# Consensys/gnark

Measured on AMD Instinct MI355X. Metric: G1 MSM throughput, BN254, 2^24 scalar-muls on one GPU (Groth16 proofs/s at 2^24 constraints in 'groth16'), higher is better.
Workload: dtype u64 Montgomery limbs in memory; 29/28-bit limbs, v_mad_u64_u32 (32x32+64) in registers

## Files before the change

gnark_amd/_lib.py:

```python
from __future__ import annotations

import ctypes as C
import os

_HERE = os.path.dirname(os.path.abspath(__file__))
DEFAULT_PATH = os.path.join(_HERE, "libgnark_amd.so")

GA_OK = 0
BN254, BLS12_381 = 0, 1
G1, G2 = 0, 1
BASES_ON_DEVICE, SCALARS_ON_DEVICE, SCALARS_MONTGOMERY, TABLE_BATCHED = 0x1, 0x2, 0x4, 0x10
RESULT_ON_DEVICE, RESULT_BITREVERSED, CHECK_CURVE_ONLY = 0x20, 0x40, 0x80
POINT_OK, POINT_OFF_CURVE, POINT_NOT_IN_SUBGROUP = 0, 1, 2
VECTOR_ON_DEVICE = BASES_ON_DEVICE
SCALE_EACH, SCALE_ONE, SCALE_POWERS = 0, 1, 2
FFT_FORWARD, FFT_INVERSE = 0, 1
DIF, DIT = 0, 1


class GnarkAmdError(RuntimeError):
    pass


class G16Key(C.Structure):
# ... 104 lines not shown
    "ga_g16_h_chain": (C.c_int, [_P, _P, C.c_uint64, _P]),
    "ga_g16_h_chain_dev": (C.c_int, [_P, _P, C.c_uint64]),
    "ga_g16_h_combine": (C.c_int, [_P, _P, _P, _P]),
    "ga_g16_z_partial": (C.c_int, [_P, _P, _P]),
    "ga_g16_prove_multi": (C.c_int, [C.POINTER(_P), C.c_uint32, _P, _P, _P, _P, C.c_uint64, C.c_uint64, _P, _P, _P]),
    "ga_g16_pk_read_mem": (C.c_int, [_P, C.c_int, _P, C.c_size_t, C.c_int32, C.c_uint32, C.c_uint32, _P, C.c_uint64, C.POINTER(_P), C.POINTER(C.c_uint64)]),
    "ga_g16_pk_read_fd": (C.c_int, [_P, C.c_int, C.c_int, C.c_int32, C.c_uint32, C.c_uint32, _P, C.c_uint64, C.POINTER(_P), C.POINTER(C.c_uint64)]),
    "ga_g16_pk_read_mem_checked": (C.c_int, [_P, C.c_int, _P, C.c_size_t, C.c_int32, C.c_uint32, C.c_uint32, _P, C.c_uint64, C.POINTER(_P), C.POINTER(C.c_uint64)]),
    "ga_g16_pk_read_fd_checked": (C.c_int, [_P, C.c_int, C.c_int, C.c_int32, C.c_uint32, C.c_uint32, _P, C.c_uint64, C.POINTER(_P), C.POINTER(C.c_uint64)]),
    "ga_g16_key_write_fd": (C.c_int, [_P, C.POINTER(G16Key), C.c_int, C.c_int, C.POINTER(C.c_uint64)]),
    "ga_g16_proof_unmarshal": (C.c_int, [C.c_int, _P, C.c_size_t, _P, _P, C.c_uint32, C.POINTER(C.c_uint32), _P, C.POINTER(C.c_size_t)]),
    "ga_point_unmarshal": (C.c_int, [C.c_int, C.c_int, _P, C.c_size_t, _P, C.POINTER(C.c_size_t)]),
    "ga_g16_proof_marshal": (C.c_int, [C.c_int, _P, _P, C.c_size_t, C.POINTER(C.c_size_t)]),
    "ga_g16_commit": (C.c_int, [_P, C.c_uint32, _P, C.c_uint64, _P, _P]),
    "ga_g16_fold_pok": (C.c_int, [C.c_int, _P, C.c_uint64, _P, _P]),
    "ga_hash_to_field": (C.c_int, [C.c_int, _P, C.c_size_t, _P, C.c_size_t, C.c_uint32, _P]),
    "ga_expand_message_xmd": (C.c_int, [_P, C.c_size_t, _P, C.c_size_t, C.c_size_t, _P]),
    "ga_g16_proof_marshal_bsb22": (C.c_int, [C.c_int, _P, _P, C.c_uint32, _P, _P, C.c_size_t, C.POINTER(C.c_size_t)]),
    "ga_g16_proof_marshal_raw": (C.c_int, [C.c_int, _P, _P, C.c_uint32, _P, _P, C.c_size_t, C.POINTER(C.c_size_t)]),
    "ga_g1_marshal_uncompressed": (C.c_int, [C.c_int, _P, _P, C.c_size_t, C.POINTER(C.c_size_t)]),
    "ga_profile_enable": (C.c_int, [_P, C.c_int]),
    "ga_profile_reset": (C.c_int, [_P]),
    "ga_profile_read": (C.c_int, [_P, C.c_char_p, C.c_size_t]),
    "ga_gen_bases": (C.c_int, [_P, C.c_int, C.c_int, C.c_uint64, C.c_size_t, _P, _P]),
    "ga_gen_bases_at": (C.c_int, [_P, C.c_int, C.c_int, C.c_uint64, C.c_uint64, C.c_size_t, _P, _P]),
    "ga_gen_scalars": (C.c_int, [_P, C.c_int, C.c_uint64, C.c_size_t, _P]),
    "ga_fr_dot": (C.c_int, [_P, C.c_int, _P, _P, C.c_size_t, _P]),
    "ga_generator_mul": (C.c_int, [C.c_int, C.c_int, _P, _P]),
    "ga_microbench": (C.c_int, [_P, C.c_char_p, C.c_size_t]),
    "ga_clock_probe": (C.c_int, [_P, C.c_uint32, C.POINTER(C.c_double)]),
}

EXPORTED_SYMBOLS = tuple(_PROTOS)


class Library:

    def __init__(self, path: str = DEFAULT_PATH):
        if not os.path.exists(path):
            raise GnarkAmdError(
                f"{path} not found: build the HIP library first "
                "(`python -c 'import __graft_entry__ as g; g.build()'` or `make -C gnark_amd/csrc -j8`). "
                "gnark_amd has no CPU fallback.")
        self.path = path
        self.dll = C.CDLL(path)
        for name, (res, args) in _PROTOS.items():
# ... 19 lines not shown
```

gnark_amd/csrc/abi.hip:

```cpp
#include <stdarg.h>
#include <stdlib.h>

#include <memory>
#include <new>
#include <vector>

#include "hostops.hip.h"

namespace ga {

static thread_local char g_err[1024] = "";

void set_error(const char* fmt, ...) {
    va_list ap;
    va_start(ap, fmt);
    vsnprintf(g_err, sizeof(g_err), fmt, ap);
    va_end(ap);
}
const char* get_error() { return g_err; }

int abi_exception_code(const char* entry) noexcept {
    try {
        throw;
    } catch (const std::bad_alloc&) {
// ... 77 lines not shown
    std::lock_guard<std::mutex> g(scratch_mu);
    auto it = scratch.find(key);
    if (it != scratch.end() && it->second.bytes >= bytes) {
        *out = it->second.p;
        return GA_OK;
    }
    if (it != scratch.end()) {
        hipFree(it->second.p);
        scratch.erase(it);
    }
    void* p = nullptr;
    const size_t slack = bytes / 8 < (64u << 20) ? bytes / 8 : (size_t)(64u << 20);
    size_t want = bytes + slack + 256;
    hipError_t e = device_malloc(&p, want);
    if (e != hipSuccess) {
        set_error("device scratch '%s': device_malloc(%zu) failed: %s", key, want, device_malloc_error(e));
        return GA_ERR_NOMEM;
    }
    scratch[key] = ScratchBuf{p, want, lane};
    *out = p;
    return GA_OK;
}

void Ctx::scratch_free_all() {
    std::lock_guard<std::mutex> g(scratch_mu);
    for (auto& kv : scratch) hipFree(kv.second.p);
    scratch.clear();
}

void Ctx::scratch_free_lanes(int first_lane) {
    std::lock_guard<std::mutex> g(scratch_mu);
    for (auto it = scratch.begin(); it != scratch.end();) {
        if (it->second.lane >= first_lane) {
            hipFree(it->second.p);
            it = scratch.erase(it);
        } else
            ++it;
    }
}

static uint64_t env_u64(const char* name, uint64_t dflt) {
    const char* e = getenv(name);
    return e ? strtoull(e, nullptr, 10) : dflt;
}
static int env_int(const char* name, int dflt) {
    const char* e = getenv(name);
// ... 16 lines not shown
    put64(g16_table_budget_pct, env_u64("GA_G16_TABLE_BUDGET_PCT", 0));
    put(g16_split, (int)env_u64("GA_G16_SPLIT", 1));
    put(g16_batch_tables, (int)env_u64("GA_G16_BATCH_TABLES", 1));
    put(ntt_wave_local, (int)env_u64("GA_NTT_WAVE_LOCAL", 1));
    put(ntt_direct, (int)env_u64("GA_NTT_DIRECT", 1));
    put(table_c, (int)env_u64("GA_TABLE_C", 0));
    put(msm_exact_redo, (int)env_u64("GA_MSM_EXACT_REDO", 0));
    put64(msm_fuse_min, env_u64("GA_MSM_FUSE_MIN", 1ull << 21));
    put64(msm_task_exact_min, env_u64("GA_MSM_TASK_EXACT_MIN", 1ull << 25));
    put(msm_xcd, (int)env_u64("GA_MSM_XCD", 3));
    {
        const uint64_t g = env_u64("GA_MSM_P1_GRID", 512);
        put64(msm_p1_grid, g ? g : 1);
    }
    {
        const char* e = getenv("GA_FAULT_THROW");
        put64(fault_throw, (e && *e) ? fnv1a(e) : 0);
    }
    put(fault_lane2_nomem, (int)env_u64("GA_FAULT_LANE2_NOMEM", 0));
    const int grp = (int)env_u64("GA_MSM_GROUP", 0);
    put(msm_group, (grp >= 2 && grp <= 256 && (grp & (grp - 1)) == 0) ? grp : 0);
    const uint64_t seg = env_u64("GA_MSM_MIN_SEG", 256);
    if (seg >= 32) put64(msm_min_seg, seg);
    g_table_c = table_c.load();
}

typedef CtxLock Lock;

static uint32_t env_segment(const char* name) {
    const uint64_t v = env_u64(name, 0);
    return (uint32_t)(v < (1u << 20) ? v : (1u << 20));
}

static bool abi_curve_ok(int curve) {
    if (curve == GA_BN254 || curve == GA_BLS12_381) return true;
    set_error("%s: unknown curve id %d", current_entry(), curve);
    return false;
}
static bool abi_curve_group_ok(int curve, int group) {
    if ((curve == GA_BN254 || curve == GA_BLS12_381) && (group == GA_G1 || group == GA_G2)) return true;
    set_error("%s: unknown curve id %d or group id %d", current_entry(), curve, group);
    return false;
}
static bool abi_range_ok(size_t n, uint64_t first) {
    if ((uint64_t)n <= (1ull << 32) && (n == 0 || first <= UINT64_MAX - (uint64_t)n + 1)) return true;
    set_error("%s: n = %zu above 2^32, or first + n above 2^64", current_entry(), n);
// ... 96 lines not shown

const char* ga_last_error(void) { return get_error(); }
const char* ga_version(void) { return "gnark_amd 0.1 (gfx950; Groth16/PLONK prover kernels: MSM G1/G2, NTT; BN254, BLS12-381)"; }

int ga_device_count(int* count) try {
    GA_ABI_ENTRY();
    GA_HIP_CHECK(hipGetDeviceCount(count));
    return GA_OK;
} GA_ABI_CATCH

int ga_ctx_create(int device, ga_ctx** out) try {
    GA_ABI_ENTRY();
    int count = 0;
    hipError_t e = hipGetDeviceCount(&count);
    if (e != hipSuccess || count <= 0) {
        set_error("no HIP device available (%s); libgnark_amd has no CPU fallback", e == hipSuccess ? "count=0" : hipGetErrorString(e));
        return GA_ERR_HIP;
    }
    if (device < 0 || device >= count) {
        set_error("device %d out of range (have %d)", device, count);
        return GA_ERR_INVALID;
    }
    GA_HIP_CHECK(hipSetDevice(device));
    {
        hipDeviceProp_t prop;
        GA_HIP_CHECK(hipGetDeviceProperties(&prop, device));
        if (prop.warpSize != 64) {
            set_error("device %d runs %d-lane wavefronts; libgnark_amd's kernels need 64 (gfx950)", device, prop.warpSize);
            return GA_ERR_INVALID;
        }
    }
    Ctx* c = new Ctx();
    c->device = device;
    hipStream_t* slots[3 + GA_NUM_LANES] = {&c->lane_stream[0], &c->lane_stream[1], &c->lane_stream[2], &c->lane_stream[3],
                                            &c->copy_stream, &c->slot_stream[0], &c->slot_stream[1]};
    for (int k = 0; k < 3 + GA_NUM_LANES; k++) {
        hipError_t se = hipStreamCreateWithFlags(slots[k], hipStreamNonBlocking);
        if (se != hipSuccess) {
            set_error("hipStreamCreate failed: %s", hipGetErrorString(se));
            for (int q = 0; q < k; q++) hipStreamDestroy(*slots[q]);
            delete c;
            return GA_ERR_HIP;
        }
    }
    c->stream = c->lane_stream[0];
    c->tun.read_env();
    *out = reinterpret_cast<ga_ctx*>(c);
    return GA_OK;
} GA_ABI_CATCH

void ga_ctx_destroy(ga_ctx* h) try {
    GA_ABI_ENTRY();
    if (!h) return;
    Ctx* c = reinterpret_cast<Ctx*>(h);
    hipSetDevice(c->device);
    for (int l = 0; l < GA_NUM_LANES; l++) hipStreamSynchronize(c->lane_stream[l]);
// ... 868 lines not shown
    }
    c->stages.clear();
    return GA_OK;
} GA_ABI_CATCH

int ga_profile_read(ga_ctx* h, char* buf, size_t cap) try {
    GA_ABI_ENTRY();
    Ctx* c = reinterpret_cast<Ctx*>(h);
    Lock l(c);
    GA_HIP_CHECK(hipStreamSynchronize(c->stream));
    std::string out;
    for (auto& s : c->stages) {
        float ms = 0;
        if (hipEventElapsedTime(&ms, s.a, s.b) != hipSuccess) ms = -1;
        char tmp[160];
        snprintf(tmp, sizeof(tmp), "%s=%.6f;", s.name.c_str(), ms);
        out += tmp;
    }
    if (!buf || cap == 0) return GA_ERR_INVALID;
    snprintf(buf, cap, "%s", out.c_str());
    return GA_OK;
} GA_ABI_CATCH

int ga_gen_bases(ga_ctx* h, int curve, int group, uint64_t seed, size_t n, void* bases_dev, void* dlogs_dev) try {
    GA_ABI_ENTRY();
    Ctx* c = reinterpret_cast<Ctx*>(h);
    Lock l(c);
    GA_DISPATCH_CURVE(curve, GA_DISPATCH_GROUP(group, GA_CHECK((util_gen_bases<C, G>(c, seed, n, bases_dev, dlogs_dev)))));
    GA_HIP_CHECK(hipStreamSynchronize(c->stream));
    return GA_OK;
} GA_ABI_CATCH

int ga_gen_bases_at(ga_ctx* h, int curve, int group, uint64_t seed, uint64_t first, size_t n, void* bases_dev, void* dlogs_dev) try {
    GA_ABI_ENTRY();
    Ctx* c = reinterpret_cast<Ctx*>(h);
    Lock l(c);
    GA_DISPATCH_CURVE(curve, GA_DISPATCH_GROUP(group, GA_CHECK((util_gen_bases<C, G>(c, seed, n, bases_dev, dlogs_dev, first)))));
    GA_HIP_CHECK(hipStreamSynchronize(c->stream));
    return GA_OK;
} GA_ABI_CATCH

int ga_gen_scalars(ga_ctx* h, int curve, uint64_t seed, size_t n, void* scalars_dev) try {
    GA_ABI_ENTRY();
    Ctx* c = reinterpret_cast<Ctx*>(h);
    Lock l(c);
    GA_DISPATCH_CURVE(curve, GA_CHECK(util_gen_scalars<C>(c, seed, n, scalars_dev)));
// ... 62 lines not shown
```

gnark_amd/csrc/common.hip.h:

```cpp
#pragma once
#include <hip/hip_runtime.h>
#include <stdint.h>
#include <stdio.h>
#include <string.h>

#include <chrono>
#include <condition_variable>
#include <atomic>
#include <map>
#include <mutex>
#include <set>
#include <string>
#include <vector>

#include "../../include/gnark_amd.h"
#include "ec.hip.h"

namespace ga {

#if defined(__HIP_DEVICE_COMPILE__) && !defined(__GFX9__)
#error "libgnark_amd: the kernels assume the 64-lane wavefronts of GFX9 / CDNA (gfx950); a wave32 target would compile and compute wrong transforms and sorts"
#endif
#define GA_REQUIRE_WAVE64() static_assert(true, "64-lane wavefronts: enforced for the whole device pass at the top of common.hip.h")

// ... 80 lines not shown
    typedef typename C::FpP P;
    GA_HD static Affine<Fe2<P>> get() {
        return {{fe_const<P>(P::G2X0), fe_const<P>(P::G2X1)}, {fe_const<P>(P::G2Y0), fe_const<P>(P::G2Y1)}};
    }
};

struct StageRec {
    std::string name;
    hipEvent_t a, b;
};

struct Tunables {
    std::atomic<uint64_t> msm_max_chunk{0};
    std::atomic<uint64_t> reduce_lazy_min{1u << 14};
    std::atomic<int> g16_share_min_pct{90};
    std::atomic<uint64_t> g16_table_budget_pct{0};
    std::atomic<int> g16_lanes{2};
    std::atomic<int> g16_split{1};
    std::atomic<int> g16_batch_tables{1};
    std::atomic<int> ntt_wave_local{1};
    std::atomic<int> ntt_direct{1};
    std::atomic<int> table_c{0};
    std::atomic<uint64_t> msm_min_seg{256};
    std::atomic<int> msm_exact_redo{0};
    std::atomic<uint64_t> msm_fuse_min{1ull << 21};
    std::atomic<int> msm_group{0};
    std::atomic<uint64_t> fault_throw{0};
    std::atomic<int> fault_lane2_nomem{0};
    std::atomic<uint64_t> msm_p1_grid{512};
    std::atomic<uint64_t> msm_task_exact_min{1ull << 25};
    std::atomic<int> msm_xcd{3};
    void read_env();
};

constexpr int GA_NUM_LANES = 4;
int current_lane();
int table_c_override();
struct LaneScope {
    int prev;
    explicit LaneScope(int lane);
    ~LaneScope();
};

struct Ctx {
    int device = 0;
    uint32_t* host_pin[GA_NUM_LANES] = {nullptr, nullptr, nullptr, nullptr};
    uint32_t* pinned_words() {
        const int l = current_lane();
        if (!host_pin[l] && hipHostMalloc((void**)&host_pin[l], 256, 0) != hipSuccess) {
            host_pin[l] = nullptr;
            (void)hipGetLastError();
        }
        return host_pin[l];
    }
    Tunables tun;
    hipStream_t stream = nullptr;
    hipStream_t lane_stream[GA_NUM_LANES] = {nullptr, nullptr, nullptr, nullptr};
    std::mutex lane_mu[GA_NUM_LANES];
    hipStream_t work_stream() const { return lane_stream[current_lane()]; }
    std::atomic<uint64_t> stat_lane0{0}, stat_lane2{0}, stat_queued{0}, stat_split{0};
    hipStream_t copy_stream = nullptr;
    std::mutex mu;
    std::mutex slot_mu;
    std::condition_variable slot_cv;
    bool slot_busy[2] = {false, false};
    hipStream_t slot_stream[2] = {nullptr, nullptr};
    std::mutex scratch_mu;
    std::atomic<int> oneshot_inflight{0};
// ... 65 lines not shown
        degenerate.insert(table);
    }
    void forget_table(const void* table) {
        std::lock_guard<std::mutex> g(degenerate_mu);
        degenerate.erase(table);
        sparse_sets.erase(table);
    }
    std::map<const void*, uint32_t> sparse_sets;
    bool is_sparse_set(const void* table) {
        std::lock_guard<std::mutex> g(degenerate_mu);
        auto it = sparse_sets.find(table);
        if (it == sparse_sets.end()) return false;
        return (++it->second % 16) != 0;
    }
    void note_sparse_set(const void* table, bool sparse) {
        std::lock_guard<std::mutex> g(degenerate_mu);
        if (sparse)
            sparse_sets.emplace(table, 0u);
        else
            sparse_sets.erase(table);
    }

    int scratch_get(const char* key, size_t bytes, void** out);
    void scratch_free_all();
    void scratch_free_lanes(int first_lane);
};

struct CtxLock {
    std::lock_guard<std::mutex> g;
    explicit CtxLock(Ctx* c) : g(c->mu) {
        hipSetDevice(c->device);
        c->tun.read_env();
    }
};

struct LaneLock {
    std::unique_lock<std::mutex> dev, l1;
    int lane = 0;
    LaneScope* scope = nullptr;
    explicit LaneLock(Ctx* c) : dev(c->mu, std::try_to_lock), l1(c->lane_mu[1], std::defer_lock) {
        hipSetDevice(c->device);
        if (!dev.owns_lock()) {
            if (!c->profiling && c->tun.g16_lanes > 1 && l1.try_lock()) lane = 1;
            else dev.lock();
        }
        if (lane == 0) c->tun.read_env();
// ... 46 lines not shown
    while ((1ull << l) < x) l++;
    return l;
}

template <class C, int G>
int msm_windows_device(Ctx* ctx, const void* d_bases, const void* d_scalars, size_t n, bool scalars_mont, int c,
                       int win_lo, int win_hi, void* h_window_sums, bool combine = false);
template <class C>
int msm_plan(int group, size_t n, int* c, int* nwin);
template <class C>
int msm_plan_table(size_t n, int* c, int* nwin, bool batched = false);

struct MsmPrepared {
    size_t n = 0;
    int c = 0, nwin = 0, win_lo = 0, win_hi = 0;
    int nsets = 0;
    bool table = false;
    uint32_t half = 0, nb = 0, seg = 0;
    uint64_t m = 0, max_tasks = 0;
    uint32_t *vals = nullptr, *task_off = nullptr, *task_start = nullptr, *task_key = nullptr, *task_perm = nullptr;
    uint32_t* task_key_by_id = nullptr;
    uint32_t* task_dest = nullptr;
};

template <class C, int G>
int msm_table_build(Ctx* ctx, const void* d_bases, size_t n, int c, void* d_table);
template <class C, int G>
size_t msm_table_point_bytes();
template <class C, int G>
int msm_table_device(Ctx* ctx, const void* d_table, const void* d_scalars, size_t n, bool scalars_mont, int c, void* h_sum, int win_lo = 0,
                     int win_hi = -1);
template <class C, int G>
int msm_table_device_batch(Ctx* ctx, const void* d_table, const void* const* d_scalars, int batch, size_t n, bool scalars_mont, int c,
                           void* h_sums);
template <class C>
int msm_prepare_table_scalars(Ctx* ctx, const void* d_scalars, size_t n, bool scalars_mont, int c, MsmPrepared* P, int slot = 0,
                              int win_lo = 0, int win_hi = -1);
template <class C, int G>
int msm_table_device_reuse(Ctx* ctx, const void* d_table, const MsmPrepared& P, void* h_sum);
template <class C, int G>
int msm_table_device_reuse_multi(Ctx* ctx, const void* const* tables, int ntab, const MsmPrepared& P, void* h_sums);

struct Domain;
template <class C> int ntt_domain_new(Ctx* ctx, uint64_t n, Domain** out);
template <class C> int ntt_domain_fft(Domain* d, void* d_data, int direction, int decimation, int on_coset);
template <class C> int ntt_domain_compute_h(Domain* d, void* d_a, void* d_b, void* d_c);
// ... 81 lines not shown
```

gnark_amd/csrc/msm_reduce.hip.h:

```cpp
#pragma once
#include <vector>

#include "msm_lazy.hip.h"

namespace ga {

constexpr int MSM_HOT_TASKS = 16;
constexpr uint32_t MSM_VHOT_TASKS = 512;
constexpr uint32_t MSM_VHOT_SPLIT = 64;
constexpr int MSM_GROUP = 32;

template <class F>
__global__ void __launch_bounds__(64)
msm_hot_kernel(const XYZZ<F>* __restrict__ partial, const uint32_t* __restrict__ task_off,
               const uint32_t* __restrict__ hot_list, const uint32_t* __restrict__ hot_count, XYZZ<F>* __restrict__ bsum,
               uint32_t bsum_stride, uint32_t part_stride) {
    __shared__ LazyPt<F> sh[64];
    __shared__ XYZZ<F> shx[64];
    __shared__ uint32_t bad;
    partial += (uint64_t)blockIdx.y * part_stride;
    bsum += (uint64_t)blockIdx.y * bsum_stride;
    const uint32_t nh = *hot_count;
    for (uint32_t h = blockIdx.x; h < nh; h += gridDim.x) {
        const uint32_t b = hot_list[h];
        const uint32_t t0 = task_off[b], t1 = task_off[b + 1];
        block_sum29<F>(t1 - t0, [&](uint32_t i) { return &partial[t0 + i]; }, &bsum[b], sh, shx, &bad);
    }
}

template <class F>
// ... 244 lines not shown
    uint32_t vtmp_stride;
};
template <class F>
int msm_merge_scratch(Ctx* ctx, const MsmPrepared& P, int ntab, hipStream_t st, MsmMerge<F>* M) {
    const uint64_t vhot_cap = P.max_tasks / MSM_VHOT_TASKS + 2;
    GA_CHECK(ctx->scratch_get("msm_hot", ((uint64_t)P.nb + 2) * 4, (void**)&M->hot_list));
    GA_CHECK(ctx->scratch_get("msm_hot_count", 256, (void**)&M->hot_count));
    GA_CHECK(ctx->scratch_get("msm_vhot", vhot_cap * 4, (void**)&M->vhot_list));
    GA_CHECK(ctx->scratch_get("msm_vhot_tmp", (uint64_t)ntab * vhot_cap * MSM_VHOT_SPLIT * sizeof(XYZZ<F>), (void**)&M->vtmp));
    M->vtmp_stride = (uint32_t)(vhot_cap * MSM_VHOT_SPLIT);
    GA_HIP_CHECK(hipMemsetAsync(M->hot_count, 0, 8, st));
    return GA_OK;
}
template <class F>
int msm_merge(Ctx* ctx, const MsmPrepared& P, int ntab, hipStream_t st, const MsmMerge<F>& M, XYZZ<F>* sums) {
    StageTimer tm(ctx, "msm_merge");
    const uint32_t nb = P.nb, part_stride = (uint32_t)P.max_tasks;
    const unsigned ny = (unsigned)ntab;
    XYZZ<F>* bsum = sums;
    const XYZZ<F>* partial = sums + (uint64_t)ntab * nb;
    const uint32_t *task_off = P.task_off, *hot_count = M.hot_count, *vhot_count = M.hot_count + 1;
    hipLaunchKernelGGL((msm_merge_kernel<F>), dim3((nb + 255) / 256, ny), dim3(256), 0, st, partial, task_off, nb, bsum, M.hot_list, M.hot_count,
                       M.vhot_list, M.hot_count + 1, part_stride);
    hipLaunchKernelGGL((msm_hot_kernel<F>), dim3(512, ny), dim3(64), 0, st, partial, task_off, (const uint32_t*)M.hot_list, hot_count, bsum, nb,
                       part_stride);
    hipLaunchKernelGGL((msm_vhot_stage1_kernel<F>), dim3(2048, ny), dim3(64), 0, st, partial, task_off, (const uint32_t*)M.vhot_list, vhot_count,
                       M.vtmp, part_stride, M.vtmp_stride);
    hipLaunchKernelGGL((msm_vhot_stage2_kernel<F>), dim3(256, ny), dim3(64), 0, st, (const XYZZ<F>*)M.vtmp, (const uint32_t*)M.vhot_list,
                       vhot_count, bsum, nb, M.vtmp_stride);
    GA_KERNEL_CHECK();
    return GA_OK;
}

template <class F>
struct MsmRows {
    const XYZZ<F>* d = nullptr;
    int per_set = 1;
    const uint32_t* flagged_groups = nullptr;
};

template <class F>
int msm_reduce_exact(Ctx* ctx, const MsmReducePlan& R, uint32_t half, const XYZZ<F>* bsum, hipStream_t st, MsmRows<F>* rows) {
    XYZZ<F>*gsum, *gsum2, *wsum;
    GA_CHECK(ctx->scratch_get("msm_gsum", (uint64_t)R.total_groups * sizeof(XYZZ<F>), (void**)&gsum));
    GA_CHECK(ctx->scratch_get("msm_gsum2", ((uint64_t)R.total_groups / 1024 + 64) * sizeof(XYZZ<F>), (void**)&gsum2));
    GA_CHECK(ctx->scratch_get("msm_wsum", (uint64_t)R.nsets * sizeof(XYZZ<F>), (void**)&wsum));
    StageTimer tm(ctx, "msm_reduce");
// ... 95 lines not shown
```

gnark_amd/csrc/msm_tasks.hip.h:

```cpp
#pragma once
#include "msm_sort.hip.h"

namespace ga {

typedef rocprim::radix_sort_config<rocprim::default_config, rocprim::default_config, rocprim::default_config, 32768> MsmTaskSort;

static __global__ void __launch_bounds__(256) msm_offsets_tasks_kernel(const uint32_t* __restrict__ keys, uint64_t m, uint32_t nb, uint32_t seg,
                                                                       uint32_t* __restrict__ off, uint32_t* __restrict__ ntask) {
    __shared__ uint32_t sh[257];
    const uint32_t b = blockIdx.x * blockDim.x + threadIdx.x;
    auto lower = [&](uint32_t key) {
        uint64_t lo = 0, hi = m;
        while (lo < hi) {
            const uint64_t mid = (lo + hi) >> 1;
            if (keys[mid] < key) lo = mid + 1;
            else hi = mid;
        }
        return (uint32_t)lo;
    };
    if (b <= nb) {
        sh[threadIdx.x] = lower(b);
        off[b] = sh[threadIdx.x];
        if (threadIdx.x == blockDim.x - 1 && b < nb) sh[blockDim.x] = lower(b + 1);
    }
    __syncthreads();
    if (b <= nb) ntask[b] = b < nb ? (sh[threadIdx.x + 1] - sh[threadIdx.x] + seg - 1) / seg : 0;
}

static __global__ void msm_tasks_kernel(const uint32_t* __restrict__ off, uint32_t nb, uint32_t seg, uint32_t* __restrict__ ntask) {
    uint32_t b = blockIdx.x * blockDim.x + threadIdx.x;
    if (b > nb) return;
    uint32_t sz = b < nb ? off[b + 1] - off[b] : 0;
    ntask[b] = (sz + seg - 1) / seg;
}

static __global__ void msm_task_init_kernel(uint32_t* __restrict__ task_qkey, uint32_t* __restrict__ task_id, uint32_t n, uint32_t* __restrict__ long_count) {
    uint32_t i = blockIdx.x * blockDim.x + threadIdx.x;
    if (i < n) {
        task_qkey[i] = 0xFFFFFFFFu;
        task_id[i] = i;
    }
    if (i == 0) *long_count = 0;
}

constexpr uint32_t MSM_LONG_TASKS = 64;
static __global__ void msm_task_list_kernel(const uint32_t* __restrict__ off, const uint32_t* __restrict__ task_off, uint32_t nb,
                                            uint32_t seg, int qshift, uint32_t* __restrict__ task_start, uint32_t* __restrict__ task_key,
                                            uint32_t* __restrict__ task_qkey, uint32_t* __restrict__ task_dest, uint32_t* __restrict__ long_list,
                                            uint32_t* __restrict__ long_count) {
    uint32_t b = blockIdx.x * blockDim.x + threadIdx.x;
    if (b >= nb) return;
    uint32_t t0 = task_off[b], t1 = task_off[b + 1];
    uint32_t start = off[b], end = off[b + 1];
    if (t1 - t0 > MSM_LONG_TASKS) {
        long_list[atomicAdd(long_count, 1u)] = b;
        return;
    }
    for (uint32_t t = t0; t < t1; t++) {
        uint32_t len = end - start < seg ? end - start : seg;
        task_start[t] = start;
        task_dest[t] = (t1 - t0 == 1) ? b : nb + t;
        task_key[t] = seg - len;
        task_qkey[t] = (seg - len) >> qshift;
        start += len;
    }
}

static __global__ void msm_task_list_long_kernel(const uint32_t* __restrict__ off, const uint32_t* __restrict__ task_off, uint32_t nb, uint32_t seg,
                                                 int qshift, uint32_t* __restrict__ task_start, uint32_t* __restrict__ task_key,
                                                 uint32_t* __restrict__ task_qkey, uint32_t* __restrict__ task_dest,
                                                 const uint32_t* __restrict__ long_list, const uint32_t* __restrict__ long_count) {
    const uint32_t nl = *long_count;
    for (uint32_t h = blockIdx.x; h < nl; h += gridDim.x) {
        const uint32_t b = long_list[h];
        const uint32_t t0 = task_off[b], t1 = task_off[b + 1];
        const uint32_t start = off[b], end = off[b + 1];
        for (uint32_t t = t0 + threadIdx.x; t < t1; t += blockDim.x) {
            const uint32_t s0 = start + (t - t0) * seg;
            const uint32_t len = end - s0 < seg ? end - s0 : seg;
            task_start[t] = s0;
            task_dest[t] = nb + t;
            task_key[t] = seg - len;
// ... 34 lines not shown
        if (want < seg) seg = want;
    }
    *end_bit = 1;
    while ((1ull << *end_bit) <= nb) (*end_bit)++;
    P->n = n;
    P->c = c;
    P->nwin = nwin;
    P->win_lo = win_lo;
    P->win_hi = win_hi;
    P->nsets = table ? batch : nwl;
    P->table = table;
    P->half = half;
    P->nb = (uint32_t)nb;
    P->seg = (uint32_t)seg;
    P->m = m;
    P->max_tasks = nb + m / P->seg + 1;
    return GA_OK;
}

inline int msm_build_tasks(Ctx* ctx, const std::string& sfx, hipStream_t st, uint32_t* off, const uint32_t* sorted_keys, MsmPrepared* P) {
    auto key = [&](const char* k) { return std::string(k) + sfx; };
    const uint32_t nb = P->nb, seg = P->seg;
    const uint64_t max_tasks = P->max_tasks;
    uint32_t *ntask, *task_off, *task_start, *task_key, *task_key2, *task_qkey, *task_id, *task_perm, *task_dest, *long_list, *long_count;
    void* tmp;
    GA_CHECK(ctx->scratch_get(key("msm_ntask").c_str(), ((uint64_t)nb + 2) * 4, (void**)&ntask));
    GA_CHECK(ctx->scratch_get(key("msm_task_off").c_str(), ((uint64_t)nb + 2) * 4, (void**)&task_off));
    GA_CHECK(ctx->scratch_get(key("msm_task_start").c_str(), max_tasks * 4, (void**)&task_start));
    GA_CHECK(ctx->scratch_get(key("msm_task_key").c_str(), max_tasks * 4, (void**)&task_key));
    GA_CHECK(ctx->scratch_get(key("msm_task_key2").c_str(), max_tasks * 4, (void**)&task_key2));
    GA_CHECK(ctx->scratch_get(key("msm_task_qkey").c_str(), max_tasks * 4, (void**)&task_qkey));
    GA_CHECK(ctx->scratch_get(key("msm_task_id").c_str(), max_tasks * 4, (void**)&task_id));
    GA_CHECK(ctx->scratch_get(key("msm_task_perm").c_str(), max_tasks * 4, (void**)&task_perm));
    GA_CHECK(ctx->scratch_get(key("msm_task_dest").c_str(), max_tasks * 4, (void**)&task_dest));
    StageTimer tm(ctx, "msm_tasks", st);
    GA_CHECK(ctx->scratch_get(key("msm_long").c_str(), (max_tasks / MSM_LONG_TASKS + 2) * 4, (void**)&long_list));
    GA_CHECK(ctx->scratch_get(key("msm_long_count").c_str(), 256, (void**)&long_count));
    int kbits = 1;
    while ((1u << kbits) <= seg) kbits++;
    const bool exact = P->m >= ctx->tun.msm_task_exact_min.load(std::memory_order_relaxed);
    const int qbits = exact || kbits < 7 ? kbits : 7, qshift = kbits - qbits;
    hipLaunchKernelGGL(msm_task_init_kernel, dim3((unsigned)((max_tasks + 255) / 256)), dim3(256), 0, st, task_qkey, task_id, (uint32_t)max_tasks, long_count);
    if (sorted_keys)
        hipLaunchKernelGGL(msm_offsets_tasks_kernel, dim3((nb + 1 + 255) / 256), dim3(256), 0, st, sorted_keys, P->m, nb, seg, off, ntask);
    else
        hipLaunchKernelGGL(msm_tasks_kernel, dim3((nb + 1 + 255) / 256), dim3(256), 0, st, (const uint32_t*)off, nb, seg, ntask);
    GA_KERNEL_CHECK();
    size_t tmp_bytes = 0;
    GA_HIP_CHECK(hipcub::DeviceScan::ExclusiveSum(nullptr, tmp_bytes, ntask, task_off, (int)(nb + 1), st));
    GA_CHECK(ctx->scratch_get(key("msm_scan_tmp").c_str(), tmp_bytes + 256, &tmp));
    GA_HIP_CHECK(hipcub::DeviceScan::ExclusiveSum(tmp, tmp_bytes, ntask, task_off, (int)(nb + 1), st));
    hipLaunchKernelGGL(msm_task_list_kernel, dim3((nb + 255) / 256), dim3(256), 0, st, (const uint32_t*)off, (const uint32_t*)task_off,
                       nb, seg, qshift, task_start, task_key, task_qkey, task_dest, long_list, long_count);
    hipLaunchKernelGGL(msm_task_list_long_kernel, dim3(256), dim3(256), 0, st, (const uint32_t*)off, (const uint32_t*)task_off, nb, seg,
                       qshift, task_start, task_key, task_qkey, task_dest, (const uint32_t*)long_list, (const uint32_t*)long_count);
    GA_KERNEL_CHECK();
    size_t tb = 0;
    GA_HIP_CHECK((rocprim::radix_sort_pairs<MsmTaskSort>(nullptr, tb, task_qkey, task_key2, task_id, task_perm, (size_t)max_tasks, 0u, (unsigned)(qbits + 1), st)));
    GA_CHECK(ctx->scratch_get(key("msm_tasksort_tmp").c_str(), tb + 256, &tmp));
    GA_HIP_CHECK((rocprim::radix_sort_pairs<MsmTaskSort>(tmp, tb, task_qkey, task_key2, task_id, task_perm, (size_t)max_tasks, 0u, (unsigned)(qbits + 1), st)));
    P->task_off = task_off;
    P->task_start = task_start;
    P->task_key = task_key2;
    P->task_key_by_id = task_key;
    P->task_perm = task_perm;
    P->task_dest = task_dest;
    return GA_OK;
}

template <class FrP>
int msm_prepare(Ctx* ctx, const void* d_scalars, size_t n, bool scalars_mont, int c, int win_lo, int win_hi, bool table,
                MsmPrepared* P, int slot = 0, int batch = 1) {
    hipStream_t st = ctx->work_stream();
    const std::string sfx = slot ? "#1" : "";
    int end_bit;
    GA_CHECK(msm_plan_prepare(ctx, FrP::BITS, n, c, win_lo, win_hi, table, batch, P, &end_bit));
// ... 9 lines not shown
```

gnark_amd/device.py:

```python
from __future__ import annotations

import ctypes as C

import numpy as np

from . import _lib

FP_LIMBS = {_lib.BN254: 4, _lib.BLS12_381: 6}
FR_LIMBS = 4
CURVE_IDS = {"bn254": _lib.BN254, "bls12-381": _lib.BLS12_381, "bls12_381": _lib.BLS12_381,
             _lib.BN254: _lib.BN254, _lib.BLS12_381: _lib.BLS12_381}


def curve_id(curve) -> int:
    try:
        return CURVE_IDS[curve]
    except KeyError:
        raise ValueError(f"unsupported curve {curve!r} (built: bn254, bls12-381)") from None


def affine_words(curve: int, group: int) -> int:
    return FP_LIMBS[curve] * (2 if group == _lib.G1 else 4)


# ... 40 lines not shown
        return {"name": name.value.decode(), "total_bytes": tot.value, "free_bytes": free.value}

    def malloc(self, nbytes: int) -> "DeviceBuffer":
        p = C.c_void_p()
        self.lib.check(self.lib.ga_malloc(self.handle, nbytes, C.byref(p)))
        return DeviceBuffer(self, p.value, nbytes)

    def to_device(self, a: np.ndarray) -> "DeviceBuffer":
        a = np.ascontiguousarray(a)
        buf = self.malloc(a.nbytes)
        if a.nbytes:
            self.lib.check(self.lib.ga_copy_to_device(self.handle, buf.ptr, _ptr(a), a.nbytes))
        return buf

    def sync(self):
        self.lib.check(self.lib.ga_sync(self.handle))

    def lane_stats(self):
        out = (C.c_uint64 * 6)()
        self.lib.check(self.lib.ga_g16_lane_stats(self.handle, out))
        keys = ("lanes01_proofs", "lanes23_proofs", "queued_proofs", "split_proofs", "lanes01_scratch_bytes", "lanes23_scratch_bytes")
        return dict(zip(keys, (int(v) for v in out)))

    def profile(self, on: bool):
        self.lib.check(self.lib.ga_profile_enable(self.handle, 1 if on else 0))
        self.profiling = bool(on)

    def profile_reset(self):
        self.lib.check(self.lib.ga_profile_reset(self.handle))

    def profile_read(self):
        buf = C.create_string_buffer(1 << 20)
        self.lib.check(self.lib.ga_profile_read(self.handle, buf, len(buf)))
        out = []
        for item in buf.value.decode().split(";"):
            if item:
                k, v = item.split("=")
                out.append((k, float(v)))
        return out

    def microbench(self):
        buf = C.create_string_buffer(4096)
        self.lib.check(self.lib.ga_microbench(self.handle, buf, len(buf)))
        return dict((k, float(v)) for k, v in (it.split("=") for it in buf.value.decode().split(";") if it))


# ... 19 lines not shown
```

include/gnark_amd.h:

```cpp
#ifndef GNARK_AMD_H
#define GNARK_AMD_H

#include <stddef.h>
#include <stdint.h>

#ifdef __cplusplus
extern "C" {
#endif

#define GA_OK 0
#define GA_ERR_INVALID (-1)
#define GA_ERR_HIP (-2)
#define GA_ERR_NOMEM (-3)
#define GA_ERR_STATE (-4)

#define GA_BN254 0
#define GA_BLS12_381 1

#define GA_G1 0
#define GA_G2 1

#define GA_BASES_ON_DEVICE 0x1u
#define GA_SCALARS_ON_DEVICE 0x2u
#define GA_TABLE_BATCHED 0x10u
// ... 209 lines not shown
                               uint32_t shard_count, const uint64_t* k_remove, uint64_t len_k_remove, ga_g16_pk** out, uint64_t* bytes_read);
int ga_g16_pk_read_fd_checked(ga_ctx* ctx, int curve, int fd, int32_t precompute, uint32_t shard_index, uint32_t shard_count,
                              const uint64_t* k_remove, uint64_t len_k_remove, ga_g16_pk** out, uint64_t* bytes_read);
int ga_g16_key_write_fd(ga_ctx* ctx, const ga_g16_key* key, int format, int fd, uint64_t* bytes_written);
int ga_g16_proof_unmarshal(int curve, const uint8_t* data, size_t len, void* proof_out, void* commitments_out,
                           uint32_t max_commitments, uint32_t* n_commitments, void* pok_out, size_t* consumed);
int ga_point_unmarshal(int curve, int group, const uint8_t* data, size_t len, void* affine_out, size_t* consumed);

int ga_g16_proof_marshal(int curve, const void* proof, uint8_t* out, size_t cap, size_t* len);

int ga_g16_commit(ga_g16_pk* pk, uint32_t index, const void* values, uint64_t n_values, void* commitment_out, void* pok_out);
int ga_g16_fold_pok(int curve, const void* poks, uint64_t n, const void* challenge, void* out);
int ga_hash_to_field(int curve, const uint8_t* msg, size_t msg_len, const uint8_t* dst, size_t dst_len, uint32_t count, void* out);
int ga_expand_message_xmd(const uint8_t* msg, size_t msg_len, const uint8_t* dst, size_t dst_len, size_t n, uint8_t* out);
int ga_g16_proof_marshal_bsb22(int curve, const void* proof, const void* commitments, uint32_t n, const void* pok,
                               uint8_t* out, size_t cap, size_t* len);
int ga_g16_proof_marshal_raw(int curve, const void* proof, const void* commitments, uint32_t n, const void* pok,
                             uint8_t* out, size_t cap, size_t* len);
int ga_g1_marshal_uncompressed(int curve, const void* affine, uint8_t* out, size_t cap, size_t* len);

int ga_profile_enable(ga_ctx* ctx, int on);
int ga_profile_reset(ga_ctx* ctx);
int ga_profile_read(ga_ctx* ctx, char* buf, size_t cap);

int ga_gen_bases(ga_ctx* ctx, int curve, int group, uint64_t seed, size_t n, void* bases_dev, void* dlogs_dev);
int ga_gen_bases_at(ga_ctx* ctx, int curve, int group, uint64_t seed, uint64_t first, size_t n, void* bases_dev, void* dlogs_dev);
int ga_gen_scalars(ga_ctx* ctx, int curve, uint64_t seed, size_t n, void* scalars_dev);
int ga_fr_dot(ga_ctx* ctx, int curve, const void* a_dev, const void* b_dev, size_t n, void* out_host);
int ga_generator_mul(int curve, int group, const void* k_canonical_le32, void* out_jac);

int ga_microbench(ga_ctx* ctx, char* buf, size_t cap);
int ga_clock_probe(ga_ctx* ctx, uint32_t micros, double* mhz_out);

#ifdef __cplusplus
}
#endif
#endif
```

Measured before the change: 880.6.

## Split a hashed subset of MSM buckets into random-sized pieces to smooth task ramp

Adds a ramp mode to MSM task generation. A hash-selected subset of buckets, sized from the CU count, is split into 2+ pieces of pseudo-random length, using spare task slots up to max_tasks. Task counts become 64-bit (plain and extra) and are scanned, then task offsets are computed inside the list kernel. The goal is to even out load imbalance and tail effects in the bucket-accumulation schedule, at the cost of extra merge work, larger scratch, and a stats entry point.

Result: no change. 883.6 (median of 6 runs) (+0.3%).

```diff
diff --git a/gnark_amd/_lib.py b/gnark_amd/_lib.py
--- a/gnark_amd/_lib.py
+++ b/gnark_amd/_lib.py
@@ -150,6 +150,7 @@
     "ga_profile_enable": (C.c_int, [_P, C.c_int]),
     "ga_profile_reset": (C.c_int, [_P]),
     "ga_profile_read": (C.c_int, [_P, C.c_char_p, C.c_size_t]),
+    "ga_msm_task_stats": (C.c_int, [_P, C.POINTER(C.c_uint64)]),
     "ga_gen_bases": (C.c_int, [_P, C.c_int, C.c_int, C.c_uint64, C.c_size_t, _P, _P]),
     "ga_gen_bases_at": (C.c_int, [_P, C.c_int, C.c_int, C.c_uint64, C.c_uint64, C.c_size_t, _P, _P]),
     "ga_gen_scalars": (C.c_int, [_P, C.c_int, C.c_uint64, C.c_size_t, _P]),
diff --git a/gnark_amd/csrc/abi.hip b/gnark_amd/csrc/abi.hip
--- a/gnark_amd/csrc/abi.hip
+++ b/gnark_amd/csrc/abi.hip
@@ -123,6 +123,12 @@
     return GA_OK;
 }
 
+void* Ctx::scratch_peek(const char* key) {
+    std::lock_guard<std::mutex> g(scratch_mu);
+    auto it = scratch.find(key);
+    return it == scratch.end() ? nullptr : it->second.p;
+}
+
 void Ctx::scratch_free_all() {
     std::lock_guard<std::mutex> g(scratch_mu);
     for (auto& kv : scratch) hipFree(kv.second.p);
@@ -185,6 +191,7 @@
     put(msm_group, (grp >= 2 && grp <= 256 && (grp & (grp - 1)) == 0) ? grp : 0);
     const uint64_t seg = env_u64("GA_MSM_MIN_SEG", 256);
     if (seg >= 32) put64(msm_min_seg, seg);
+    put64(msm_ramp, env_u64("GA_MSM_RAMP", 1));
     g_table_c = table_c.load();
 }
 
@@ -327,6 +334,7 @@
         return GA_ERR_INVALID;
     }
     GA_HIP_CHECK(hipSetDevice(device));
+    int cus = 0;
     {
         hipDeviceProp_t prop;
         GA_HIP_CHECK(hipGetDeviceProperties(&prop, device));
@@ -334,9 +342,11 @@
             set_error("device %d runs %d-lane wavefronts; libgnark_amd's kernels need 64 (gfx950)", device, prop.warpSize);
             return GA_ERR_INVALID;
         }
+        cus = prop.multiProcessorCount;
     }
     Ctx* c = new Ctx();
     c->device = device;
+    c->cus = cus > 0 ? cus : 1;
     hipStream_t* slots[3 + GA_NUM_LANES] = {&c->lane_stream[0], &c->lane_stream[1], &c->lane_stream[2], &c->lane_stream[3],
                                             &c->copy_stream, &c->slot_stream[0], &c->slot_stream[1]};
     for (int k = 0; k < 3 + GA_NUM_LANES; k++) {
@@ -1251,6 +1261,24 @@
     return GA_OK;
 } GA_ABI_CATCH
 
+int ga_msm_task_stats(ga_ctx* h, uint64_t* out8) try {
+    GA_ABI_ENTRY();
+    Ctx* c = reinterpret_cast<Ctx*>(h);
+    if (!c || !out8) {
+        set_error("ga_msm_task_stats: null argument");
+        return GA_ERR_INVALID;
+    }
+    Lock l(c);
+    GA_HIP_CHECK(hipStreamSynchronize(c->stream));
+    const char* sets[2] = {"msm_long_count", "msm_long_count#1"};
+    for (int s = 0; s < 2; s++) {
+        uint32_t w[4] = {0, 0, 0, 0};
+        if (const void* p = c->scratch_peek(sets[s])) GA_HIP_CHECK(hipMemcpy(w, (const uint32_t*)p + MSM_STAT_WORD, sizeof(w), hipMemcpyDeviceToHost));
+        for (int k = 0; k < 4; k++) out8[4 * s + k] = w[k];
+    }
+    return GA_OK;
+} GA_ABI_CATCH
+
 int ga_gen_bases(ga_ctx* h, int curve, int group, uint64_t seed, size_t n, void* bases_dev, void* dlogs_dev) try {
     GA_ABI_ENTRY();
     Ctx* c = reinterpret_cast<Ctx*>(h);
diff --git a/gnark_amd/csrc/common.hip.h b/gnark_amd/csrc/common.hip.h
--- a/gnark_amd/csrc/common.hip.h
+++ b/gnark_amd/csrc/common.hip.h
@@ -126,6 +126,7 @@
     std::atomic<int> ntt_direct{1};
     std::atomic<int> table_c{0};
     std::atomic<uint64_t> msm_min_seg{256};
+    std::atomic<uint64_t> msm_ramp{1};
     std::atomic<int> msm_exact_redo{0};
     std::atomic<uint64_t> msm_fuse_min{1ull << 21};
     std::atomic<int> msm_group{0};
@@ -148,6 +149,7 @@
 
 struct Ctx {
     int device = 0;
+    int cus = 0;
     uint32_t* host_pin[GA_NUM_LANES] = {nullptr, nullptr, nullptr, nullptr};
     uint32_t* pinned_words() {
         const int l = current_lane();
@@ -259,6 +261,7 @@
     }
 
     int scratch_get(const char* key, size_t bytes, void** out);
+    void* scratch_peek(const char* key);
     void scratch_free_all();
     void scratch_free_lanes(int first_lane);
 };
@@ -351,6 +354,8 @@
     uint32_t* task_key_by_id = nullptr;
     uint32_t* task_dest = nullptr;
 };
+
+constexpr int MSM_STAT_WORD = 4;
 
 template <class C, int G>
 int msm_table_build(Ctx* ctx, const void* d_bases, size_t n, int c, void* d_table);
diff --git a/gnark_amd/csrc/msm_reduce.hip.h b/gnark_amd/csrc/msm_reduce.hip.h
--- a/gnark_amd/csrc/msm_reduce.hip.h
+++ b/gnark_amd/csrc/msm_reduce.hip.h
@@ -5,7 +5,13 @@
 
 namespace ga {
 
-constexpr int MSM_HOT_TASKS = 16;
+#ifndef GA_MSM_HOT_TASKS
+#define GA_MSM_HOT_TASKS 16
+#endif
+#ifndef GA_MSM_HOT_GRID
+#define GA_MSM_HOT_GRID 512
+#endif
+constexpr int MSM_HOT_TASKS = GA_MSM_HOT_TASKS;
 constexpr uint32_t MSM_VHOT_TASKS = 512;
 constexpr uint32_t MSM_VHOT_SPLIT = 64;
 constexpr int MSM_GROUP = 32;
@@ -296,7 +302,7 @@
     const uint32_t *task_off = P.task_off, *hot_count = M.hot_count, *vhot_count = M.hot_count + 1;
     hipLaunchKernelGGL((msm_merge_kernel<F>), dim3((nb + 255) / 256, ny), dim3(256), 0, st, partial, task_off, nb, bsum, M.hot_list, M.hot_count,
                        M.vhot_list, M.hot_count + 1, part_stride);
-    hipLaunchKernelGGL((msm_hot_kernel<F>), dim3(512, ny), dim3(64), 0, st, partial, task_off, (const uint32_t*)M.hot_list, hot_count, bsum, nb,
+    hipLaunchKernelGGL((msm_hot_kernel<F>), dim3(GA_MSM_HOT_GRID, ny), dim3(64), 0, st, partial, task_off, (const uint32_t*)M.hot_list, hot_count, bsum, nb,
                        part_stride);
     hipLaunchKernelGGL((msm_vhot_stage1_kernel<F>), dim3(2048, ny), dim3(64), 0, st, partial, task_off, (const uint32_t*)M.vhot_list, vhot_count,
                        M.vtmp, part_stride, M.vtmp_stride);
diff --git a/gnark_amd/csrc/msm_tasks.hip.h b/gnark_amd/csrc/msm_tasks.hip.h
--- a/gnark_amd/csrc/msm_tasks.hip.h
+++ b/gnark_amd/csrc/msm_tasks.hip.h
@@ -5,8 +5,44 @@
 
 typedef rocprim::radix_sort_config<rocprim::default_config, rocprim::default_config, rocprim::default_config, 32768> MsmTaskSort;
 
+#ifndef GA_MSM_RAMP_PIECES
+#define GA_MSM_RAMP_PIECES 2
+#endif
+#ifndef GA_MSM_RAMP_K_MUL
+#define GA_MSM_RAMP_K_MUL 1
+#endif
+static_assert(GA_MSM_RAMP_PIECES >= 2 && GA_MSM_RAMP_PIECES <= 16, "a split bucket's pieces are summed by the merge kernel's lane");
+struct MsmRamp {
+    uint32_t k = 0, min_tasks = 0, cap = 0, pieces = GA_MSM_RAMP_PIECES;
+};
+GA_HD uint32_t msm_mix(uint32_t x) {
+    x *= 0x9E3779B1u;
+    x ^= x >> 15;
+    x *= 0x85EBCA77u;
+    x ^= x >> 13;
+    x *= 0xC2B2AE3Du;
+    x ^= x >> 16;
+    return x;
+}
+GA_HD bool msm_ramp_marks(const MsmRamp& rp, uint32_t b, uint32_t sz, uint32_t seg) {
+    return rp.k != 0 && sz >= 2 && sz <= seg && (msm_mix(b >> 6) & (rp.k - 1)) == 0;
+}
+GA_HD uint32_t msm_ramp_piece(uint32_t b, uint32_t i, uint32_t left, uint32_t after) {
+    return after == 0 ? left : 1 + msm_mix((b << 4 | i) ^ 0x5BD1E995u) % (left - after);
+}
+GA_HD uint64_t msm_task_count(const MsmRamp& rp, uint32_t b, uint32_t sz, uint32_t seg) {
+    const uint32_t extra = msm_ramp_marks(rp, b, sz, seg) ? (sz < rp.pieces ? sz : rp.pieces) - 1 : 0;
+    return (uint64_t)((sz + seg - 1) / seg) | ((uint64_t)extra << 32);
+}
+GA_HD uint32_t msm_ramp_allowed(const MsmRamp& rp, uint64_t totals, uint32_t max_tasks) {
+    const uint32_t plain = (uint32_t)totals, marked = (uint32_t)(totals >> 32);
+    if (rp.k == 0 || plain < rp.min_tasks || plain >= max_tasks) return 0;
+    uint32_t a = marked < rp.cap ? marked : rp.cap;
+    return a < max_tasks - plain ? a : max_tasks - plain;
+}
+
 static __global__ void __launch_bounds__(256) msm_offsets_tasks_kernel(const uint32_t* __restrict__ keys, uint64_t m, uint32_t nb, uint32_t seg,
-                                                                       uint32_t* __restrict__ off, uint32_t* __restrict__ ntask) {
+                                                                       const MsmRamp rp, uint32_t* __restrict__ off, uint64_t* __restrict__ ntask) {
     __shared__ uint32_t sh[257];
     const uint32_t b = blockIdx.x * blockDim.x + threadIdx.x;
     auto lower = [&](uint32_t key) {
@@ -24,14 +60,13 @@
         if (threadIdx.x == blockDim.x - 1 && b < nb) sh[blockDim.x] = lower(b + 1);
     }
     __syncthreads();
-    if (b <= nb) ntask[b] = b < nb ? (sh[threadIdx.x + 1] - sh[threadIdx.x] + seg - 1) / seg : 0;
-}
-
-static __global__ void msm_tasks_kernel(const uint32_t* __restrict__ off, uint32_t nb, uint32_t seg, uint32_t* __restrict__ ntask) {
+    if (b <= nb) ntask[b] = b < nb ? msm_task_count(rp, b, sh[threadIdx.x + 1] - sh[threadIdx.x], seg) : 0;
+}
+
+static __global__ void msm_tasks_kernel(const uint32_t* __restrict__ off, uint32_t nb, uint32_t seg, const MsmRamp rp, uint64_t* __restrict__ ntask) {
     uint32_t b = blockIdx.x * blockDim.x + threadIdx.x;
     if (b > nb) return;
-    uint32_t sz = b < nb ? off[b + 1] - off[b] : 0;
-    ntask[b] = (sz + seg - 1) / seg;
+    ntask[b] = b < nb ? msm_task_count(rp, b, off[b + 1] - off[b], seg) : 0;
 }
 
 static __global__ void msm_task_init_kernel(uint32_t* __restrict__ task_qkey, uint32_t* __restrict__ task_id, uint32_t n, uint32_t* __restrict__ long_count) {
@@ -44,20 +79,37 @@
 }
 
 constexpr uint32_t MSM_LONG_TASKS = 64;
-static __global__ void msm_task_list_kernel(const uint32_t* __restrict__ off, const uint32_t* __restrict__ task_off, uint32_t nb,
-                                            uint32_t seg, int qshift, uint32_t* __restrict__ task_start, uint32_t* __restrict__ task_key,
+static __global__ void msm_task_list_kernel(const uint32_t* __restrict__ off, const uint64_t* __restrict__ count_scan, uint32_t nb,
+                                            uint32_t seg, int qshift, const MsmRamp rp, uint32_t max_tasks, uint32_t* __restrict__ task_off,
+                                            uint32_t* __restrict__ task_start, uint32_t* __restrict__ task_key,
                                             uint32_t* __restrict__ task_qkey, uint32_t* __restrict__ task_dest, uint32_t* __restrict__ long_list,
                                             uint32_t* __restrict__ long_count) {
     uint32_t b = blockIdx.x * blockDim.x + threadIdx.x;
-    if (b >= nb) return;
-    uint32_t t0 = task_off[b], t1 = task_off[b + 1];
+    if (b > nb) return;
+    const uint64_t totals = count_scan[nb];
+    const uint32_t allowed = msm_ramp_allowed(rp, totals, max_tasks);
+    const uint64_t s0 = count_scan[b];
+    const uint32_t r0 = (uint32_t)(s0 >> 32) < allowed ? (uint32_t)(s0 >> 32) : allowed;
+    const uint32_t t0 = (uint32_t)s0 + r0;
+    task_off[b] = t0;
+    if (b == nb) {
+        long_count[MSM_STAT_WORD] = t0;
+        long_count[MSM_STAT_WORD + 1] = max_tasks;
+        long_count[MSM_STAT_WORD + 2] = (uint32_t)(totals >> 32);
+        long_count[MSM_STAT_WORD + 3] = allowed;
+        return;
+    }
+    const uint64_t s1 = count_scan[b + 1];
+    const uint32_t r1 = (uint32_t)(s1 >> 32) < allowed ? (uint32_t)(s1 >> 32) : allowed;
+    const uint32_t t1 = (uint32_t)s1 + r1;
     uint32_t start = off[b], end = off[b + 1];
-    if (t1 - t0 > MSM_LONG_TASKS) {
+    if ((uint32_t)s1 - (uint32_t)s0 > MSM_LONG_TASKS) {
         long_list[atomicAdd(long_count, 1u)] = b;
         return;
     }
+    const bool split = r1 != r0;
     for (uint32_t t = t0; t < t1; t++) {
-        uint32_t len = end - start < seg ? end - start : seg;
+        uint32_t len = split ? msm_ramp_piece(b, t - t0, end - start, t1 - 1 - t) : end - start < seg ? end - start : seg;
         task_start[t] = start;
         task_dest[t] = (t1 - t0 == 1) ? b : nb + t;
         task_key[t] = seg - len;
@@ -138,9 +190,11 @@
     auto key = [&](const char* k) { return std::string(k) + sfx; };
     const uint32_t nb = P->nb, seg = P->seg;
     const uint64_t max_tasks = P->max_tasks;
-    uint32_t *ntask, *task_off, *task_start, *task_key, *task_key2, *task_qkey, *task_id, *task_perm, *task_dest, *long_list, *long_count;
+    uint32_t *task_off, *task_start, *task_key, *task_key2, *task_qkey, *task_id, *task_perm, *task_dest, *long_list, *long_count;
+    uint64_t *ntask, *count_scan;
     void* tmp;
-    GA_CHECK(ctx->scratch_get(key("msm_ntask").c_str(), ((uint64_t)nb + 2) * 4, (void**)&ntask));
+    GA_CHECK(ctx->scratch_get(key("msm_ntask").c_str(), ((uint64_t)nb + 2) * 8, (void**)&ntask));
+    GA_CHECK(ctx->scratch_get(key("msm_count_scan").c_str(), ((uint64_t)nb + 2) * 8, (void**)&count_scan));
     GA_CHECK(ctx->scratch_get(key("msm_task_off").c_str(), ((uint64_t)nb + 2) * 4, (void**)&task_off));
     GA_CHECK(ctx->scratch_get(key("msm_task_start").c_str(), max_tasks * 4, (void**)&task_start));
     GA_CHECK(ctx->scratch_get(key("msm_task_key").c_str(), max_tasks * 4, (void**)&task_key));
@@ -156,18 +210,28 @@
     while ((1u << kbits) <= seg) kbits++;
     const bool exact = P->m >= ctx->tun.msm_task_exact_min.load(std::memory_order_relaxed);
     const int qbits = exact || kbits < 7 ? kbits : 7, qshift = kbits - qbits;
+    MsmRamp rp;
+    const uint64_t ramp = ctx->tun.msm_ramp.load(std::memory_order_relaxed), resident = (uint64_t)(ctx->cus > 0 ? ctx->cus : 1) * 16 * 64;
+    const uint64_t ramp_min = ramp == 1 ? 4 * resident : ramp;
+    if (ramp != 0 && max_tasks >= ramp_min) {
+        rp.k = 1;
+        while (2ull * rp.k * resident <= nb) rp.k *= 2;
+        rp.k *= GA_MSM_RAMP_K_MUL;
+        rp.min_tasks = (uint32_t)ramp_min;
+        rp.cap = (uint32_t)(max_tasks - nb);
+    }
     hipLaunchKernelGGL(msm_task_init_kernel, dim3((unsigned)((max_tasks + 255) / 256)), dim3(256), 0, st, task_qkey, task_id, (uint32_t)max_tasks, long_count);
     if (sorted_keys)
-        hipLaunchKernelGGL(msm_offsets_tasks_kernel, dim3((nb + 1 + 255) / 256), dim3(256), 0, st, sorted_keys, P->m, nb, seg, off, ntask);
+        hipLaunchKernelGGL(msm_offsets_tasks_kernel, dim3((nb + 1 + 255) / 256), dim3(256), 0, st, sorted_keys, P->m, nb, seg, rp, off, ntask);
     else
-        hipLaunchKernelGGL(msm_tasks_kernel, dim3((nb + 1 + 255) / 256), dim3(256), 0, st, (const uint32_t*)off, nb, seg, ntask);
+        hipLaunchKernelGGL(msm_tasks_kernel, dim3((nb + 1 + 255) / 256), dim3(256), 0, st, (const uint32_t*)off, nb, seg, rp, ntask);
     GA_KERNEL_CHECK();
     size_t tmp_bytes = 0;
-    GA_HIP_CHECK(hipcub::DeviceScan::ExclusiveSum(nullptr, tmp_bytes, ntask, task_off, (int)(nb + 1), st));
+    GA_HIP_CHECK(hipcub::DeviceScan::ExclusiveSum(nullptr, tmp_bytes, ntask, count_scan, (int)(nb + 1), st));
     GA_CHECK(ctx->scratch_get(key("msm_scan_tmp").c_str(), tmp_bytes + 256, &tmp));
-    GA_HIP_CHECK(hipcub::DeviceScan::ExclusiveSum(tmp, tmp_bytes, ntask, task_off, (int)(nb + 1), st));
-    hipLaunchKernelGGL(msm_task_list_kernel, dim3((nb + 255) / 256), dim3(256), 0, st, (const uint32_t*)off, (const uint32_t*)task_off,
-                       nb, seg, qshift, task_start, task_key, task_qkey, task_dest, long_list, long_count);
+    GA_HIP_CHECK(hipcub::DeviceScan::ExclusiveSum(tmp, tmp_bytes, ntask, count_scan, (int)(nb + 1), st));
+    hipLaunchKernelGGL(msm_task_list_kernel, dim3((nb + 1 + 255) / 256), dim3(256), 0, st, (const uint32_t*)off, (const uint64_t*)count_scan,
+                       nb, seg, qshift, rp, (uint32_t)max_tasks, task_off, task_start, task_key, task_qkey, task_dest, long_list, long_count);
     hipLaunchKernelGGL(msm_task_list_long_kernel, dim3(256), dim3(256), 0, st, (const uint32_t*)off, (const uint32_t*)task_off, nb, seg,
                        qshift, task_start, task_key, task_qkey, task_dest, (const uint32_t*)long_list, (const uint32_t*)long_count);
     GA_KERNEL_CHECK();
diff --git a/gnark_amd/device.py b/gnark_amd/device.py
--- a/gnark_amd/device.py
+++ b/gnark_amd/device.py
@@ -86,6 +86,13 @@
         keys = ("lanes01_proofs", "lanes23_proofs", "queued_proofs", "split_proofs", "lanes01_scratch_bytes", "lanes23_scratch_bytes")
         return dict(zip(keys, (int(v) for v in out)))
 
+    def msm_task_stats(self, witness_set=False):
+        out = (C.c_uint64 * 8)()
+        self.lib.check(self.lib.ga_msm_task_stats(self.handle, out))
+        keys = ("tasks", "max_tasks", "ramp_selected", "ramp_split")
+        first = 4 if witness_set else 0
+        return dict(zip(keys, (int(v) for v in out[first:first + 4])))
+
     def profile(self, on: bool):
         self.lib.check(self.lib.ga_profile_enable(self.handle, 1 if on else 0))
         self.profiling = bool(on)
diff --git a/include/gnark_amd.h b/include/gnark_amd.h
--- a/include/gnark_amd.h
+++ b/include/gnark_amd.h
@@ -255,6 +255,7 @@
 int ga_profile_enable(ga_ctx* ctx, int on);
 int ga_profile_reset(ga_ctx* ctx);
 int ga_profile_read(ga_ctx* ctx, char* buf, size_t cap);
+int ga_msm_task_stats(ga_ctx* ctx, uint64_t* out8);
 
 int ga_gen_bases(ga_ctx* ctx, int curve, int group, uint64_t seed, size_t n, void* bases_dev, void* dlogs_dev);
 int ga_gen_bases_at(ga_ctx* ctx, int curve, int group, uint64_t seed, uint64_t first, size_t n, void* bases_dev, void* dlogs_dev);
```
